# SunYangtian/UniGeo

Measured on AMD Instinct MI355X. Metric: frames/sec (384x512, 25-frame clip, 25 denoise steps), higher is better.
Workload: dtype fp16; 1 GPU; DepthCrafter SVD-UNet fp16, 25-step Euler, 25-frame 384x512 clips (BASELINE configs[1]); CLIP + VAE enc/dec + depth post-proc inside the timed region; one clip per ug_dc_run call, one call at a time (SURVEY 8d; reference eval.py:33-39); frames=25, height=384, width=512, denoise_steps=25, parallelism=clip-sharded x1, RCCL all_gather of depth, clips_in_flight_per_gpu=1, lanes=1

## Files before the change

unigeo_amd/csrc/kernels/ff_fused.hip:

```cpp
#include "../common.h"
#include <algorithm>
#include <type_traits>

typedef const __attribute__((address_space(1))) void* gptr_t;
typedef __attribute__((address_space(3))) void* lptr_t;
typedef float f32x2 __attribute__((ext_vector_type(2)));
typedef unsigned u32x4_t __attribute__((ext_vector_type(4)));

__device__ __forceinline__ f32x2 ff_geglu2(f32x2 h, f32x2 g) {
  const f32x2 ag = {__builtin_fabsf(g.x), __builtin_fabsf(g.y)};
  const f32x2 u = ag * 0.23164189f + 1.0f;
  const f32x2 t = {__builtin_amdgcn_rcpf(u.x), __builtin_amdgcn_rcpf(u.y)};
  f32x2 y = t * 0.5307027145f - 0.7265760135f;
  y = y * t + 0.7107068705f;
  y = y * t - 0.142248368f;
  y = y * t + 0.127414796f;
  y = y * t;
  const f32x2 w = (g * g) * -0.72134752044f;
  const f32x2 e = {__builtin_amdgcn_exp2f(w.x), __builtin_amdgcn_exp2f(w.y)};
  const f32x2 q = 0.5f - y * e;
  const f32x2 phi = {0.5f + __builtin_copysignf(q.x, g.x), 0.5f + __builtin_copysignf(q.y, g.y)};
  return h * g * phi;
}

__device__ __forceinline__ int ffswz(int row) { return (row >> 1) & 7; }

template <int KT, int ABL = 0, bool XT = false>
__global__ __launch_bounds__(512, 2) void ff_fused_kernel(const FFusedP p) {
  constexpr int C = KT * 64;
  constexpr int NP = (C + 127) / 128;
  constexpr int NPF = C / 128;
  constexpr bool TAIL = (C % 128) != 0;
  constexpr int STEPS = KT + NP;
  constexpr int TILE = 128 * 64;
  extern __shared__ __attribute__((aligned(16))) f16 smem[];
  f16* Xs = smem;
  f16* ring = smem + KT * TILE;
  f16* Gs = ring + 3 * TILE;

  const int tid = threadIdx.x, lane = tid & 63;
  const int wave = __builtin_amdgcn_readfirstlane(tid >> 6);
  const int wm = wave >> 1, wn = wave & 1;
  const int l15 = lane & 15, g = lane >> 4;
  const int sw = ffswz(l15);
  const int pc = lane & 7, lrow = lane >> 3;
  const int I = 4 * C;
  const int nchunk = I / 64;
  const int ntiles = (p.M + 127) / 128;

  constexpr unsigned SENT = 0x80000000u;
  const __amdgpu_buffer_rsrc_t rW1 = __builtin_amdgcn_make_buffer_rsrc((void*)p.W1, 0, (int)SENT, 0x00020000);
  const __amdgpu_buffer_rsrc_t rW2 = __builtin_amdgcn_make_buffer_rsrc((void*)p.W2, 0, (int)SENT, 0x00020000);
  const __amdgpu_buffer_rsrc_t rX = __builtin_amdgcn_make_buffer_rsrc((void*)p.X, 0, (int)((long)p.M * C * 2), 0x00020000);
  unsigned vo1[2], vo2[2], vot, vox;
#pragma unroll
  for (int u = 0; u < 2; ++u) {
    const int lr = (wave * 2 + u) * 8 + lrow;
    const int part = lr >> 6, rem = lr & 63, jj = rem >> 4, i = rem & 15;
    const int n = part * 64 + (i >> 2) * 16 + jj * 4 + (i & 3);
    vo1[u] = (unsigned)((n * C + (pc ^ ffswz(lr)) * 8) * 2);
    vo2[u] = (unsigned)((n * I + (pc ^ ffswz(lr)) * 8) * 2);
  }
  {
    const int lr = wave * 8 + lrow;
    const int part = lr >> 5, rem = lr & 31, jj = rem >> 4, i = rem & 15;
    const int n = NPF * 128 + part * 32 + (i >> 2) * 8 + jj * 4 + (i & 3);
    vot = (unsigned)((n * I + (pc ^ ffswz(lr)) * 8) * 2);
  }
  vox = (unsigned)((lrow * C + 0) * 2);
  auto issue_packet = [&](int j, int s, int slot) {
    f16* dst = ring + slot * TILE;
    if (s < KT) {
      const int so = (j * 128 * C + s * 64) * 2;
#pragma unroll
      for (int u = 0; u < 2; ++u)
        __builtin_amdgcn_raw_ptr_buffer_load_lds(rW1, (lptr_t)(dst + (wave * 2 + u) * 8 * 64), 16, (int)vo1[u], so, 0, 0);
    } else if (s - KT < NPF) {
      const int so = ((s - KT) * 128 * I + j * 64) * 2;
#pragma unroll
      for (int u = 0; u < 2; ++u)
        __builtin_amdgcn_raw_ptr_buffer_load_lds(rW2, (lptr_t)(dst + (wave * 2 + u) * 8 * 64), 16, (int)vo2[u], so, 0, 0);
    } else {
      __builtin_amdgcn_raw_ptr_buffer_load_lds(rW2, (lptr_t)(dst + wave * 8 * 64), 16, (int)vot, j * 64 * 2, 0, 0);
    }
  };
  auto nload = [](int s) { return (TAIL && s == STEPS - 1) ? 1 : 2; };

  static_assert(!XT || (KT >= 2 && NP >= 2), "cross-tile prefetch needs two phase-B packets after the last phase A");
  constexpr int NX = KT * 2;
  auto issue_x = [&](int m0_) {
    for (int t = wave; t < KT * 16; t += 8) {
      const int kt = t >> 4, r = t & 15;
      const int lr = r * 8 + lrow;
      const unsigned vo = vox + (unsigned)((r * 8 * C + (pc ^ ffswz(lr)) * 8) * 2);
      __builtin_amdgcn_raw_ptr_buffer_load_lds(rX, (lptr_t)(Xs + kt * TILE + r * 8 * 64), 16, (int)vo, (m0_ * C + kt * 64) * 2, 0, 0);
    }
  };
  int slot = 0;
  if (XT && (int)blockIdx.x < ntiles) { issue_x(blockIdx.x * 128); issue_packet(0, 0, 0); issue_packet(0, 1, 1); }

  for (int tile = blockIdx.x; tile < ntiles; tile += gridDim.x) {
    const int m0 = tile * 128;
    const bool more = XT && tile + (int)gridDim.x < ntiles;
    if (!XT) {
      issue_x(m0);
      issue_packet(0, 0, 0);
      issue_packet(0, 1, 1);
      slot = 0;
    }

    if (p.ln_g) {
      const int row = tid >> 2, q4 = tid & 3;
      const long mr = (long)m0 + row < p.M ? (long)m0 + row : (long)p.M - 1;
      const f16* av = p.addvec ? p.addvec + (long)((int)mr / p.rows_per_vec) * C : nullptr;
      f16x8 ga[KT][2], be[KT][2], ad[KT][2];
#pragma unroll
      for (int kt = 0; kt < KT; ++kt)
#pragma unroll
        for (int u = 0; u < 2; ++u) {
          ga[kt][u] = *(const f16x8*)(p.ln_g + kt * 64 + q4 * 16 + u * 8);
          be[kt][u] = *(const f16x8*)(p.ln_b + kt * 64 + q4 * 16 + u * 8);
          if (av) ad[kt][u] = *(const f16x8*)(av + kt * 64 + q4 * 16 + u * 8);
        }
      asm volatile("s_waitcnt vmcnt(0)" ::: "memory");
      __builtin_amdgcn_s_barrier();
      asm volatile("" ::: "memory");
      f16* xr = Xs + row * 64;
      const int cs[2] = {((q4 * 2) ^ ffswz(row)) * 8, ((q4 * 2 + 1) ^ ffswz(row)) * 8};
      f16x8 hx[KT][2];
      float sum = 0.f;
#pragma unroll
      for (int kt = 0; kt < KT; ++kt)
#pragma unroll
        for (int u = 0; u < 2; ++u) {
          hx[kt][u] = *(const f16x8*)(xr + kt * TILE + cs[u]);
          if (av) {
#pragma unroll
            for (int e = 0; e < 8; ++e) hx[kt][u][e] = (f16)((float)hx[kt][u][e] + (float)ad[kt][u][e]);
          }
#pragma unroll
          for (int e = 0; e < 8; ++e) sum += (float)hx[kt][u][e];
        }
      sum += __shfl_xor(sum, 1); sum += __shfl_xor(sum, 2);
      const float mean = sum / C;
      float var = 0.f;
#pragma unroll
      for (int kt = 0; kt < KT; ++kt)
#pragma unroll
        for (int u = 0; u < 2; ++u)
#pragma unroll
          for (int e = 0; e < 8; ++e) { const float d = (float)hx[kt][u][e] - mean; var += d * d; }
      var += __shfl_xor(var, 1); var += __shfl_xor(var, 2);
      const float rstd = rsqrtf(var / C + p.ln_eps);
#pragma unroll
      for (int kt = 0; kt < KT; ++kt)
#pragma unroll
        for (int u = 0; u < 2; ++u) {
          f16x8 y;
#pragma unroll
          for (int e = 0; e < 8; ++e) y[e] = (f16)(((float)hx[kt][u][e] - mean) * rstd * (float)ga[kt][u][e] + (float)be[kt][u][e]);
          *(f16x8*)(xr + kt * TILE + cs[u]) = y;
        }
      asm volatile("s_waitcnt lgkmcnt(0)" ::: "memory");
    }

    f32x4 acc1[2][4], acc2[NP][2][4];
#pragma unroll
    for (int i = 0; i < 2; ++i)
#pragma unroll
      for (int jn = 0; jn < 4; ++jn) {
        acc1[i][jn] = (f32x4){0.f, 0.f, 0.f, 0.f};
#pragma unroll
        for (int pp = 0; pp < NP; ++pp) acc2[pp][i][jn] = (f32x4){0.f, 0.f, 0.f, 0.f};
      }

    bool first = true;
    for (int j = 0; j < nchunk; ++j) {
#pragma unroll
      for (int s = 0; s < STEPS; ++s) {
        const bool last = (j == nchunk - 1) && (s == STEPS - 1);
        if (XT && more && j == nchunk - 1 && s > KT && s <= KT + 2) {
          if (s == KT + 1) { if (nload((KT + 2) % STEPS) == 1) asm volatile("s_waitcnt vmcnt(%0)" :: "n"(NX + 1) : "memory"); else asm volatile("s_waitcnt vmcnt(%0)" :: "n"(NX + 2) : "memory"); }
          else { if (KT + 3 < STEPS && nload(KT + 3) == 1) asm volatile("s_waitcnt vmcnt(%0)" :: "n"(NX + 1) : "memory"); else asm volatile("s_waitcnt vmcnt(%0)" :: "n"(NX + 2) : "memory"); }
        }
        else if (first || (last && !more)) asm volatile("s_waitcnt vmcnt(0)" ::: "memory");
        else if (nload((s + 1) % STEPS) == 1) asm volatile("s_waitcnt vmcnt(1)" ::: "memory");
        else asm volatile("s_waitcnt vmcnt(2)" ::: "memory");
        if (first) {
          first = false;
        }
        if (s == KT) asm volatile("s_waitcnt lgkmcnt(0)" ::: "memory");
        if (!(ABL & 16)) __builtin_amdgcn_s_barrier();
        asm volatile("" ::: "memory");
        if (!(ABL & 2)) {
          int s2 = s + 2, j2 = j;
          if (s2 >= STEPS) { s2 -= STEPS; ++j2; }
          int slot2 = slot + 2; if (slot2 >= 3) slot2 -= 3;
          if (j2 < nchunk) issue_packet(j2, s2, slot2);
          else if (more) issue_packet(0, s2, slot2);
        }
        if (XT && more && j == nchunk - 1 && s == KT) issue_x(m0 + (int)gridDim.x * 128);
        const f16* Wt = ring + slot * TILE;
        if (++slot == 3) slot = 0;
        if (s < KT) {
          const f16* Ab = Xs + s * TILE + (wm * 32 + l15) * 64;
          const f16* Bb = Wt + (wn * 64 + l15) * 64;
#pragma unroll
          for (int kk = 0; kk < 2; ++kk) {
            const int ch = ((kk * 4 + g) ^ sw) * 8;
            f16x8 bf[4], af[2];
#pragma unroll
            for (int jn = 0; jn < 4; ++jn) bf[jn] = (ABL & 8) ? (f16x8){(f16)(float)(lane + s + jn), 0, 0, 0, 0, 0, 0, 0} : *(const f16x8*)(Bb + jn * 16 * 64 + ch);
#pragma unroll
            for (int i = 0; i < 2; ++i) af[i] = (ABL & 8) ? (f16x8){(f16)(float)(lane + i), 0, 0, 0, 0, 0, 0, 0} : *(const f16x8*)(Ab + i * 16 * 64 + ch);
#pragma unroll
            for (int i = 0; i < 2; ++i)
#pragma unroll
              for (int jn = 0; jn < 4; ++jn) {
                if (ABL & 4) acc1[i][jn][0] += (float)bf[jn][0] * (float)af[i][0];
                else acc1[i][jn] = __builtin_amdgcn_mfma_f32_16x16x32_f16(bf[jn], af[i], acc1[i][jn], 0, 0, 0);
              }
          }
          if (s == KT - 1) {
            const f16x8 b0 = *(const f16x8*)(p.b1 + j * 128 + wn * 64 + g * 16), b1v = *(const f16x8*)(p.b1 + j * 128 + wn * 64 + g * 16 + 8);
#pragma unroll
            for (int i = 0; i < 2; ++i) {
              float v[16];
#pragma unroll
              for (int jn = 0; jn < 4; ++jn)
#pragma unroll
                for (int r = 0; r < 4; ++r) v[jn * 4 + r] = acc1[i][jn][r] + (float)(jn < 2 ? b0[jn * 4 + r] : b1v[(jn - 2) * 4 + r]);
              f16x8 o;
#pragma unroll
              for (int e = 0; e < 8; e += 2) {
                const f32x2 r2 = (ABL & 1) ? (f32x2){v[e] + v[8 + e], v[e + 1] + v[9 + e]} : ff_geglu2((f32x2){v[e], v[e + 1]}, (f32x2){v[8 + e], v[9 + e]});
                o[e] = (f16)r2.x; o[e + 1] = (f16)r2.y;
              }
              const int row = wm * 32 + i * 16 + l15;
              *(f16x8*)(Gs + row * 64 + (((wn * 4 + g) ^ ffswz(row)) * 8)) = o;
#pragma unroll
              for (int jn = 0; jn < 4; ++jn) acc1[i][jn] = (f32x4){0.f, 0.f, 0.f, 0.f};
            }
          }
        } else {
          const int pp = s - KT;
          const f16* Ab = Gs + (wm * 32 + l15) * 64;
          const bool tailp = TAIL && pp == NP - 1;
          const f16* Bb = Wt + ((tailp ? wn * 32 : wn * 64) + l15) * 64;
#pragma unroll
          for (int kk = 0; kk < 2; ++kk) {
            const int ch = ((kk * 4 + g) ^ sw) * 8;
            f16x8 bf[4], af[2];
#pragma unroll
            for (int jn = 0; jn < 4; ++jn)
              if (!tailp || jn < 2) bf[jn] = (ABL & 8) ? (f16x8){(f16)(float)(lane + s + jn), 0, 0, 0, 0, 0, 0, 0} : *(const f16x8*)(Bb + jn * 16 * 64 + ch);
#pragma unroll
            for (int i = 0; i < 2; ++i) af[i] = (ABL & 8) ? (f16x8){(f16)(float)(lane + i), 0, 0, 0, 0, 0, 0, 0} : *(const f16x8*)(Ab + i * 16 * 64 + ch);
#pragma unroll
            for (int i = 0; i < 2; ++i)
#pragma unroll
              for (int jn = 0; jn < 4; ++jn)
                if (!tailp || jn < 2) {
                  if (ABL & 4) acc2[pp][i][jn][0] += (float)bf[jn][0] * (float)af[i][0];
                  else acc2[pp][i][jn] = __builtin_amdgcn_mfma_f32_16x16x32_f16(bf[jn], af[i], acc2[pp][i][jn], 0, 0, 0);
                }
          }
        }
      }
    }

#pragma unroll
    for (int pp = 0; pp < NP; ++pp) {
      const bool tailp = TAIL && pp == NP - 1;
      const int wid = tailp ? 8 : 16;
      const int n0 = pp * 128 + (tailp ? wn * 32 + g * 8 : wn * 64 + g * 16);
#pragma unroll
      for (int i = 0; i < 2; ++i) {
        const int m = m0 + wm * 32 + i * 16 + l15;
        if (m >= p.M) continue;
#pragma unroll
        for (int e0 = 0; e0 < 16; e0 += 8) {
          if (e0 >= wid) continue;
          const f16x8 b = p.b2 ? *(const f16x8*)(p.b2 + n0 + e0) : (f16x8){0, 0, 0, 0, 0, 0, 0, 0};
          float o[8];
#pragma unroll
          for (int q = 0; q < 8; ++q) o[q] = p.c0 * (acc2[pp][i][(e0 + q) >> 2][(e0 + q) & 3] + (float)b[q]);
          if (p.R1) {
            f16x8 r = *(const f16x8*)(p.R1 + (long)m * C + n0 + e0);
            if (p.ln_g && p.addvec) {
              const f16x8 a = *(const f16x8*)(p.addvec + ((long)m / p.rows_per_vec) * C + n0 + e0);
#pragma unroll
              for (int q = 0; q < 8; ++q) r[q] = (f16)((float)r[q] + (float)a[q]);
            }
#pragma unroll
            for (int q = 0; q < 8; ++q) o[q] += p.c1 * (float)r[q];
          }
          if (p.R2) {
            const f16x8 r = *(const f16x8*)(p.R2 + (long)m * C + n0 + e0);
#pragma unroll
            for (int q = 0; q < 8; ++q) o[q] += p.c2 * (float)r[q];
          }
          f16x8 h;
#pragma unroll
          for (int q = 0; q < 8; ++q) h[q] = (f16)o[q];
          *(f16x8*)(p.Out + (long)m * C + n0 + e0) = h;
        }
      }
    }
    if (!XT) {
      asm volatile("s_waitcnt vmcnt(0)" ::: "memory");
      __builtin_amdgcn_s_barrier();
    }
  }
}

template <int KT>
static void launch_ff_t(const FFusedP& p, hipStream_t s) {
  const size_t lds = (size_t)(KT + 3 + 1) * 128 * 64 * sizeof(f16);
  static bool attr[32] = {};
  bool& at = attr[ug_dev_slot()];
  if (!at) { UG_CHECK(hipFuncSetAttribute((const void*)ff_fused_kernel<KT>, hipFuncAttributeMaxDynamicSharedMemorySize, (int)lds)); at = true; }
  const int ntiles = (p.M + 127) / 128;
  const int variant = p.variant;
#ifdef UG_EXPERIMENTS
  if (variant >= 100) {
    if constexpr (KT == 5) {
      auto go = [&](auto kern) {
        UG_CHECK(hipFuncSetAttribute((const void*)kern, hipFuncAttributeMaxDynamicSharedMemorySize, (int)lds));
        hipLaunchKernelGGL(kern, dim3(std::min(ntiles, 256)), dim3(512), lds, s, p);
      };
      switch (variant - 100) {
        case 1: go(ff_fused_kernel<5, 1>); break;  case 2: go(ff_fused_kernel<5, 2>); break;   case 4: go(ff_fused_kernel<5, 4>); break;
        case 8: go(ff_fused_kernel<5, 8>); break;  case 16: go(ff_fused_kernel<5, 16>); break; case 12: go(ff_fused_kernel<5, 12>); break;
        case 3: go(ff_fused_kernel<5, 3>); break;  case 14: go(ff_fused_kernel<5, 14>); break; case 30: go(ff_fused_kernel<5, 30>); break;
        case 31: go(ff_fused_kernel<5, 31>); break; case 18: go(ff_fused_kernel<5, 18>); break; case 10: go(ff_fused_kernel<5, 10>); break;
        default: go(ff_fused_kernel<5, 0>); break;
      }
      return;
    }
  }
#else
  UG_REQUIRE(variant < 100, "ff_fused: the ablation variants (100 + mask) exist only in the UG_EXPERIMENTS build (make experiments -> build/exp/libunigeo_exp.so, UG_LIB_PATH)");
#endif
  if (variant == 0) {
    if constexpr (KT >= 2 && (KT * 64 + 127) / 128 >= 2) {
      static bool attrx[32] = {};
      bool& atx = attrx[ug_dev_slot()];
      if (!atx) { UG_CHECK(hipFuncSetAttribute((const void*)ff_fused_kernel<KT, 0, true>, hipFuncAttributeMaxDynamicSharedMemorySize, (int)lds)); atx = true; }
      const int per_cu_x = std::max(1, std::min(2, (int)((160 * 1024) / lds)));
      hipLaunchKernelGGL((ff_fused_kernel<KT, 0, true>), dim3(std::min(ntiles, per_cu_x * 256)), dim3(512), lds, s, p);
      return;
    }
  }
  const int per_cu = std::max(1, std::min(2, (int)((160 * 1024) / lds)));
  const int grid = std::min(ntiles, per_cu * 256);
  hipLaunchKernelGGL(ff_fused_kernel<KT>, dim3(grid), dim3(512), lds, s, p);
}

bool ff_fused_supported(int C) { return C == 64 || C == 128 || C == 192 || C == 256 || C == 320; }

void launch_ff_fused(const FFusedP& p, hipStream_t s) {
  UG_REQUIRE(ff_fused_supported(p.C) && p.M > 0 && p.zero, "ff_fused: C must be a multiple of 64 up to 320");
  if (p.ln_g) UG_REQUIRE(p.ln_b && (!p.addvec || p.rows_per_vec >= 1) && (!p.addvec || !p.R1 || p.R1 == p.X), "ff_fused pre-norm: beta missing / residual is not the normalised stream");
  switch (p.C / 64) {
    case 1: launch_ff_t<1>(p, s); break;
    case 2: launch_ff_t<2>(p, s); break;
    case 3: launch_ff_t<3>(p, s); break;
    case 4: launch_ff_t<4>(p, s); break;
    default: launch_ff_t<5>(p, s); break;
  }
  UG_CHECK(hipGetLastError());
}
```

Measured before the change: 28.08 frames/s.

## Software-pipeline GEGLU of chunk j into second-GEMM steps of chunk j-1

Adds a PIPE variant of the fused feed-forward kernel that double-buffers the GEGLU activation tile in LDS. The GEGLU math for the next chunk is spread across the second-GEMM steps of the previous chunk and interleaved with MFMAs via sched_group_barrier. This hides the VALU activation work behind matrix instructions instead of running it serially between the two GEMMs. It makes PIPE the default for KT>=2, at the cost of one extra LDS tile, which may reduce occupancy for large C.

```diff
diff --git a/unigeo_amd/csrc/kernels/ff_fused.hip b/unigeo_amd/csrc/kernels/ff_fused.hip
--- a/unigeo_amd/csrc/kernels/ff_fused.hip
+++ b/unigeo_amd/csrc/kernels/ff_fused.hip
@@ -22,10 +22,31 @@
   const f32x2 phi = {0.5f + __builtin_copysignf(q.x, g.x), 0.5f + __builtin_copysignf(q.y, g.y)};
   return h * g * phi;
 }
+__device__ __forceinline__ float ff_geglu1(float h, float g) {
+  const float u = __builtin_fabsf(g) * 0.23164189f + 1.0f;
+  const float t = __builtin_amdgcn_rcpf(u);
+  float y = t * 0.5307027145f - 0.7265760135f;
+  y = y * t + 0.7107068705f;
+  y = y * t - 0.142248368f;
+  y = y * t + 0.127414796f;
+  y = y * t;
+  const float w = (g * g) * -0.72134752044f;
+  const float e = __builtin_amdgcn_exp2f(w);
+  const float q = 0.5f - y * e;
+  const float phi = 0.5f + __builtin_copysignf(q, g);
+  return h * g * phi;
+}
 
 __device__ __forceinline__ int ffswz(int row) { return (row >> 1) & 7; }
 
-template <int KT, int ABL = 0, bool XT = false>
+template <int I, int N, typename F>
+__device__ __forceinline__ void ff_unroll(F&& f) {
+  if constexpr (I < N) { f(std::integral_constant<int, I>{}); ff_unroll<I + 1, N>(f); }
+}
+constexpr int ff_unit_lo(int pp, int NP) { return pp >= NP ? 8 : (4 * pp < 8 ? 4 * pp : 8); }
+constexpr int FF_UNIT_VALU = 40;
+
+template <int KT, int ABL = 0, bool XT = false, bool PIPE = false>
 __global__ __launch_bounds__(512, 2) void ff_fused_kernel(const FFusedP p) {
   constexpr int C = KT * 64;
   constexpr int NP = (C + 127) / 128;
@@ -37,6 +58,7 @@
   f16* Xs = smem;
   f16* ring = smem + KT * TILE;
   f16* Gs = ring + 3 * TILE;
+  static_assert(!PIPE || ABL == 0, "the ablations are variants of the round-2 schedule");
 
   const int tid = threadIdx.x, lane = tid & 63;
   const int wave = __builtin_amdgcn_readfirstlane(tid >> 6);
@@ -175,6 +197,7 @@
       }
 
     bool first = true;
+    if constexpr (!PIPE) {
     for (int j = 0; j < nchunk; ++j) {
 #pragma unroll
       for (int s = 0; s < STEPS; ++s) {
@@ -268,6 +291,123 @@
         }
       }
     }
+    } else {
+      auto phase_a = [&](int s, const f16* Wt) {
+        const f16* Ab = Xs + s * TILE + (wm * 32 + l15) * 64;
+        const f16* Bb = Wt + (wn * 64 + l15) * 64;
+#pragma unroll
+        for (int kk = 0; kk < 2; ++kk) {
+          const int ch = ((kk * 4 + g) ^ sw) * 8;
+          f16x8 bf[4], af[2];
+#pragma unroll
+          for (int jn = 0; jn < 4; ++jn) bf[jn] = *(const f16x8*)(Bb + jn * 16 * 64 + ch);
+#pragma unroll
+          for (int i = 0; i < 2; ++i) af[i] = *(const f16x8*)(Ab + i * 16 * 64 + ch);
+#pragma unroll
+          for (int i = 0; i < 2; ++i)
+#pragma unroll
+            for (int jn = 0; jn < 4; ++jn) acc1[i][jn] = __builtin_amdgcn_mfma_f32_16x16x32_f16(bf[jn], af[i], acc1[i][jn], 0, 0, 0);
+        }
+      };
+      auto phase_b = [&](int pp, const f16* Wt, const f16* G) {
+        const f16* Ab = G + (wm * 32 + l15) * 64;
+        const bool tailp = TAIL && pp == NP - 1;
+        const f16* Bb = Wt + ((tailp ? wn * 32 : wn * 64) + l15) * 64;
+#pragma unroll
+        for (int kk = 0; kk < 2; ++kk) {
+          const int ch = ((kk * 4 + g) ^ sw) * 8;
+          f16x8 bf[4], af[2];
+#pragma unroll
+          for (int jn = 0; jn < 4; ++jn)
+            if (!tailp || jn < 2) bf[jn] = *(const f16x8*)(Bb + jn * 16 * 64 + ch);
+#pragma unroll
+          for (int i = 0; i < 2; ++i) af[i] = *(const f16x8*)(Ab + i * 16 * 64 + ch);
+#pragma unroll
+          for (int i = 0; i < 2; ++i)
+#pragma unroll
+            for (int jn = 0; jn < 4; ++jn)
+              if (!tailp || jn < 2) acc2[pp][i][jn] = __builtin_amdgcn_mfma_f32_16x16x32_f16(bf[jn], af[i], acc2[pp][i][jn], 0, 0, 0);
+        }
+      };
+      auto next_packet = [&](int& jj, int& ss) {
+        if (++ss == STEPS || (jj == 0 && ss == KT)) { ++jj; ss = jj == nchunk ? KT : 0; }
+      };
+      f16x8 bv, bg, o[2];
+      auto geglu_unit = [&](int q, f16* G) {
+        const int i = q >> 2, e = (q & 3) * 2;
+#pragma unroll
+        for (int k = 0; k < 2; ++k) {
+          const float h = acc1[i][e >> 2][(e & 3) + k] + (float)bv[e + k];
+          const float gt = acc1[i][2 + (e >> 2)][(e & 3) + k] + (float)bg[e + k];
+          o[i][e + k] = (f16)ff_geglu1(h, gt);
+        }
+        if ((q & 3) == 3) {
+          const int row = wm * 32 + i * 16 + l15;
+          *(f16x8*)(G + row * 64 + (((wn * 4 + g) ^ ffswz(row)) * 8)) = o[i];
+#pragma unroll
+          for (int jn = 0; jn < 4; ++jn) acc1[i][jn] = (f32x4){0.f, 0.f, 0.f, 0.f};
+        }
+      };
+      auto step = [&](int j, auto S, auto FIN) {
+          constexpr int s = decltype(S)::value;
+          constexpr bool fin = decltype(FIN)::value;
+          if (j == 0 && s >= KT) return;
+          int jn1 = j, sn1 = s;
+          next_packet(jn1, sn1);
+          const bool last = jn1 > nchunk;
+          const bool one = TAIL && !last && sn1 == STEPS - 1;
+          if (first || (last && !more)) asm volatile("s_waitcnt vmcnt(0)" ::: "memory");
+          else if (XT && more && j == nchunk && s > KT && s <= KT + 2) {
+            if (one) asm volatile("s_waitcnt vmcnt(%0)" :: "n"(NX + 1) : "memory"); else asm volatile("s_waitcnt vmcnt(%0)" :: "n"(NX + 2) : "memory");
+          }
+          else if (one) asm volatile("s_waitcnt vmcnt(1)" ::: "memory");
+          else asm volatile("s_waitcnt vmcnt(2)" ::: "memory");
+          first = false;
+          if (j > 0 && s == (j == nchunk ? KT : 0)) asm volatile("s_waitcnt lgkmcnt(0)" ::: "memory");
+          __builtin_amdgcn_s_barrier();
+          asm volatile("" ::: "memory");
+          if (s == KT - 1) {
+            bv = *(const f16x8*)(p.b1 + j * 128 + wn * 64 + g * 16);
+            bg = *(const f16x8*)(p.b1 + j * 128 + wn * 64 + g * 16 + 8);
+          }
+          {
+            int j2 = jn1, s2 = sn1;
+            next_packet(j2, s2);
+            int slot2 = slot + 2; if (slot2 >= 3) slot2 -= 3;
+            if (j2 <= nchunk) issue_packet(s2 < KT ? j2 : j2 - 1, s2, slot2);
+            else if (more) issue_packet(0, s2, slot2);
+          }
+          if (XT && more && j == nchunk && s == KT) issue_x(m0 + (int)gridDim.x * 128);
+          const f16* Wt = ring + slot * TILE;
+          if (++slot == 3) slot = 0;
+          if constexpr (s < KT) {
+            phase_a(s, Wt);
+            if (s == KT - 1 && j == 0) {
+#pragma unroll
+              for (int q = 0; q < 8; ++q) geglu_unit(q, Gs);
+            }
+          } else {
+            constexpr int pp = s - KT;
+            phase_b(pp, Wt, Gs + ((j - 1) & 1) * TILE);
+            if constexpr (!fin && ff_unit_lo(pp + 1, NP) > ff_unit_lo(pp, NP)) {
+              constexpr bool tailp = TAIL && pp == NP - 1;
+              constexpr int NM = tailp ? 8 : 16, NR = tailp ? 8 : 12;
+              constexpr int Q0 = ff_unit_lo(pp, NP), Q1 = ff_unit_lo(pp + 1, NP);
+              constexpr int NV = (FF_UNIT_VALU * (Q1 - Q0) + NM - 1) / NM;
+#pragma unroll
+              for (int q = Q0; q < Q1; ++q) geglu_unit(q, Gs + (j & 1) * TILE);
+              __builtin_amdgcn_sched_group_barrier(0x100, NR, 0);
+#pragma unroll
+              for (int m = 0; m < NM; ++m) {
+                __builtin_amdgcn_sched_group_barrier(0x008, 1, 0);
+                __builtin_amdgcn_sched_group_barrier(0x002, NV, 0);
+              }
+            }
+          }
+      };
+      for (int j = 0; j < nchunk; ++j) ff_unroll<0, STEPS>([&](auto S) { step(j, S, std::false_type{}); });
+      ff_unroll<KT, STEPS>([&](auto S) { step(nchunk, S, std::true_type{}); });
+    }
 
 #pragma unroll
     for (int pp = 0; pp < NP; ++pp) {
@@ -314,27 +454,32 @@
   }
 }
 
+template <int KT, int ABL, bool XT, bool PIPE>
+static void ff_launch(const FFusedP& p, hipStream_t s) {
+  constexpr size_t lds = (size_t)(KT + 3 + (PIPE ? 2 : 1)) * 128 * 64 * sizeof(f16);
+  static bool attr[32] = {};
+  bool& at = attr[ug_dev_slot()];
+  if (!at) { UG_CHECK(hipFuncSetAttribute((const void*)ff_fused_kernel<KT, ABL, XT, PIPE>, hipFuncAttributeMaxDynamicSharedMemorySize, (int)lds)); at = true; }
+  const int ntiles = (p.M + 127) / 128;
+  const int per_cu = std::max(1, std::min(2, (int)((160 * 1024) / lds)));
+  hipLaunchKernelGGL((ff_fused_kernel<KT, ABL, XT, PIPE>), dim3(std::min(ntiles, per_cu * 256)), dim3(512), lds, s, p);
+}
+
 template <int KT>
 static void launch_ff_t(const FFusedP& p, hipStream_t s) {
-  const size_t lds = (size_t)(KT + 3 + 1) * 128 * 64 * sizeof(f16);
-  static bool attr[32] = {};
-  bool& at = attr[ug_dev_slot()];
-  if (!at) { UG_CHECK(hipFuncSetAttribute((const void*)ff_fused_kernel<KT>, hipFuncAttributeMaxDynamicSharedMemorySize, (int)lds)); at = true; }
-  const int ntiles = (p.M + 127) / 128;
+  constexpr bool XT_OK = KT >= 2 && (KT * 64 + 127) / 128 >= 2;
   const int variant = p.variant;
 #ifdef UG_EXPERIMENTS
   if (variant >= 100) {
     if constexpr (KT == 5) {
-      auto go = [&](auto kern) {
-        UG_CHECK(hipFuncSetAttribute((const void*)kern, hipFuncAttributeMaxDynamicSharedMemorySize, (int)lds));
-        hipLaunchKernelGGL(kern, dim3(std::min(ntiles, 256)), dim3(512), lds, s, p);
-      };
       switch (variant - 100) {
-        case 1: go(ff_fused_kernel<5, 1>); break;  case 2: go(ff_fused_kernel<5, 2>); break;   case 4: go(ff_fused_kernel<5, 4>); break;
-        case 8: go(ff_fused_kernel<5, 8>); break;  case 16: go(ff_fused_kernel<5, 16>); break; case 12: go(ff_fused_kernel<5, 12>); break;
-        case 3: go(ff_fused_kernel<5, 3>); break;  case 14: go(ff_fused_kernel<5, 14>); break; case 30: go(ff_fused_kernel<5, 30>); break;
-        case 31: go(ff_fused_kernel<5, 31>); break; case 18: go(ff_fused_kernel<5, 18>); break; case 10: go(ff_fused_kernel<5, 10>); break;
-        default: go(ff_fused_kernel<5, 0>); break;
+        case 1: ff_launch<5, 1, false, false>(p, s); break;   case 2: ff_launch<5, 2, false, false>(p, s); break;
+        case 4: ff_launch<5, 4, false, false>(p, s); break;   case 8: ff_launch<5, 8, false, false>(p, s); break;
+        case 16: ff_launch<5, 16, false, false>(p, s); break; case 12: ff_launch<5, 12, false, false>(p, s); break;
+        case 3: ff_launch<5, 3, false, false>(p, s); break;   case 14: ff_launch<5, 14, false, false>(p, s); break;
+        case 30: ff_launch<5, 30, false, false>(p, s); break; case 31: ff_launch<5, 31, false, false>(p, s); break;
+        case 18: ff_launch<5, 18, false, false>(p, s); break; case 10: ff_launch<5, 10, false, false>(p, s); break;
+        default: ff_launch<5, 0, false, false>(p, s); break;
       }
       return;
     }
@@ -342,19 +487,13 @@
 #else
   UG_REQUIRE(variant < 100, "ff_fused: the ablation variants (100 + mask) exist only in the UG_EXPERIMENTS build (make experiments -> build/exp/libunigeo_exp.so, UG_LIB_PATH)");
 #endif
-  if (variant == 0) {
-    if constexpr (KT >= 2 && (KT * 64 + 127) / 128 >= 2) {
-      static bool attrx[32] = {};
-      bool& atx = attrx[ug_dev_slot()];
-      if (!atx) { UG_CHECK(hipFuncSetAttribute((const void*)ff_fused_kernel<KT, 0, true>, hipFuncAttributeMaxDynamicSharedMemorySize, (int)lds)); atx = true; }
-      const int per_cu_x = std::max(1, std::min(2, (int)((160 * 1024) / lds)));
-      hipLaunchKernelGGL((ff_fused_kernel<KT, 0, true>), dim3(std::min(ntiles, per_cu_x * 256)), dim3(512), lds, s, p);
-      return;
-    }
-  }
-  const int per_cu = std::max(1, std::min(2, (int)((160 * 1024) / lds)));
-  const int grid = std::min(ntiles, per_cu * 256);
-  hipLaunchKernelGGL(ff_fused_kernel<KT>, dim3(grid), dim3(512), lds, s, p);
+  if constexpr (KT >= 2) {
+    if (variant == 0) { ff_launch<KT, 0, XT_OK, true>(p, s); return; }
+  }
+  if constexpr (XT_OK) {
+    if (variant == 0 || variant == 2) { ff_launch<KT, 0, true, false>(p, s); return; }
+  }
+  ff_launch<KT, 0, false, false>(p, s);
 }
 
 bool ff_fused_supported(int C) { return C == 64 || C == 128 || C == 192 || C == 256 || C == 320; }
```

Result: no change. 28.24 frames/s, median of 6 (+0.6%).
